# pingooio/pingoo

Measured on AMD Instinct MI355X. Metric: requests/sec matched (whole node), 1k-rule WAF, higher is better.
Workload: dtype u8

## Files before the change

include/pwaf.h:

```cpp
#ifndef PWAF_H
#define PWAF_H

#include <stddef.h>
#include <stdint.h>

#ifdef __cplusplus
extern "C" {
#endif

#define PWAF_ABI_VERSION 4u

#define PWAF_OK 0
#define PWAF_E_INVALID_ARG (-1)
#define PWAF_E_SYNTAX (-2)
#define PWAF_E_UNSUPPORTED (-3)
#define PWAF_E_LIST (-4)
#define PWAF_E_DEVICE (-5)
#define PWAF_E_BATCH (-6)
#define PWAF_E_NOMEM (-7)
#define PWAF_E_BUSY (-8)
#define PWAF_W_PARTIAL 1

#define PWAF_ACTION_ALLOW 0u
#define PWAF_ACTION_BLOCK 1u
// ... 417 lines not shown

typedef struct pwaf_kernel_time {
    char name[48];
    float ms;
    uint64_t alg_bytes;
} pwaf_kernel_time;
int pwaf_engine_set_profiling(pwaf_engine *, int on);
int pwaf_engine_kernel_times(pwaf_engine *, pwaf_kernel_time *out, int cap);

typedef struct pwaf_stats {
    uint32_t n_rules, n_atoms, n_scan_atoms, n_numeric_atoms;
    uint32_t n_dfa_groups, n_dfa_states_total, max_dfa_states, dfa_table_bytes_total;
    uint32_t n_ip_lists, ipset_trie_nodes, geo_trie_nodes, n_dnf_literals;
    uint32_t n_warnings, n_filtered_groups ,
        n_gated_groups ,
        n_confirm_literals ;
} pwaf_stats;
int pwaf_engine_stats(const pwaf_engine *, pwaf_stats *out);
int pwaf_engine_rule_errors(pwaf_engine *, uint64_t *counts, size_t n_rules);
int pwaf_engine_residual_mode(const pwaf_engine *);
const char *pwaf_engine_residual_fallback(const pwaf_engine *);
size_t pwaf_program_residual_source(const pwaf_program *, int kind, char *buf, size_t cap);
long pwaf_program_residual_compile(const pwaf_program *, const char *arch, char *err, size_t err_len);
int pwaf_program_confirm_field(const pwaf_program *, uint32_t group, const uint8_t *bytes, size_t len, uint32_t arena_offset,
                               uint16_t *atoms, size_t cap, size_t *n_atoms, int *flagged, int *walk);
int pwaf_program_confirm_shape(const pwaf_program *, uint32_t group, uint32_t out[8]);
size_t pwaf_program_flat_image(const pwaf_program *, uint32_t group, uint32_t tier, uint8_t *buf, size_t cap);
#define PWAF_LIST_SCAN_WORDS 16
int pwaf_program_list_scans(const pwaf_program *, uint32_t *out, size_t cap, size_t *n_descs);
int pwaf_program_verdict_shape(const pwaf_program *, uint32_t out[8]);
uint32_t pwaf_engine_compute_units(const pwaf_engine *);
int pwaf_engine_address_tables(const pwaf_engine *, uint32_t out[8]);
int pwaf_engine_coarse_tables(const pwaf_engine *, uint32_t out[16]);
#define PWAF_FILTER_SLAB_ROWS 128
int pwaf_engine_filter_flags(pwaf_engine *, uint32_t group, uint32_t info[8], uint64_t *rows, size_t cap_rows, uint32_t *per_slab, uint32_t *pair_base, size_t cap_slabs);
int pwaf_program_stats(const pwaf_program *, pwaf_stats *out);

size_t pwaf_derive_path(const uint8_t *uri_path, size_t len);
void pwaf_derive_user_agent(const uint8_t *hdr, size_t len, int present, size_t *out_start, size_t *out_len);
void pwaf_derive_host(const uint8_t *uri_host, size_t uri_host_len, int uri_host_present,
                      const uint8_t *host_hdr, size_t host_hdr_len, int host_hdr_present,
                      int *out_from_header, size_t *out_start, size_t *out_len);

const char *pwaf_last_error(void);
uint32_t pwaf_abi_version(void);

#ifdef __cplusplus
}
#endif
#endif
```

pingoo_amd/csrc/attr.hip:

```cpp
#include <hip/hip_runtime.h>

#include <algorithm>
#include <cstdlib>

#include "kernels.h"
#include "wave.h"

namespace pwaf {

static constexpr uint32_t DIR_ESCAPE = 0x80000000u;

__device__ __forceinline__ uint32_t ip_byte(const uint32_t w[4], uint32_t k) {
    uint32_t word = k < 4 ? w[0] : k < 8 ? w[1] : k < 12 ? w[2] : w[3];
    return (word >> ((k & 3) * 8)) & 0xFFu;
}

template <bool PACKED, bool COARSE>
__global__ __launch_bounds__(COARSE ? 1024 : 256, COARSE ? 8 : 1) void ipres_kernel(VerdictArgs a) {
    constexpr uint32_t U = 4;
    extern __shared__ uint4 ipres_lds[];
    const bool from_row = a.asn == nullptr;
#ifdef PWAF_PROFILING
    const bool dir = a.dir_chunks != nullptr && !((a.debug_skip >> 16) & 1u);
    const bool skip_v6 = (a.debug_skip >> 17) & 1u, skip_v4 = (a.debug_skip >> 16) & 1u;
#else
    const bool dir = a.dir_chunks != nullptr;
    constexpr bool skip_v6 = false, skip_v4 = false;
#endif
    const uint32_t T = gridDim.x * blockDim.x;
    uint32_t i0 = blockIdx.x * blockDim.x + threadIdx.x;
    uint4 raw[U];
    uint32_t v6b[U];
    auto load_inputs = [&](uint32_t base) {
#pragma unroll
        for (uint32_t u = 0; u < U; u++) {
            const uint32_t j = base + u * T < a.n ? base + u * T : base;
            raw[u] = *reinterpret_cast<const uint4 *>(a.ip + (size_t)j * 16);
            v6b[u] = a.ip_is_v6[j];
        }
    };
    bool loaded = false;
    if (COARSE) {
        load_inputs(i0 < a.n ? i0 : 0u);
        loaded = true;
        const uint4 *src = reinterpret_cast<const uint4 *>(a.dir_coarse);
        const uint32_t n16 = a.dir_coarse_bytes >> 4;
        for (uint32_t j = threadIdx.x; j < n16; j += 4u * blockDim.x) {
            uint4 w[4];
#pragma unroll
            for (uint32_t q = 0; q < 4; q++) w[q] = src[min(j + q * blockDim.x, n16 - 1u)];
#pragma unroll
            for (uint32_t q = 0; q < 4; q++)
                if (j + q * blockDim.x < n16) ipres_lds[j + q * blockDim.x] = w[q];
        }
        __syncthreads();
    }
    for (; i0 < a.n; i0 += T * U) {
        uint32_t idx[U], ipw[U][4], eg[U], ei[U], k[U];
        bool live[U], v6[U], geo_walk[U], chunked[U];
        if (!loaded) load_inputs(i0);
        loaded = false;
#pragma unroll
        for (uint32_t u = 0; u < U; u++) {
            idx[u] = i0 + u * T;
            live[u] = idx[u] < a.n;
        }
        uint32_t first[U], top16[U];
#pragma unroll
        for (uint32_t u = 0; u < U; u++) {
            ipw[u][0] = raw[u].x; ipw[u][1] = raw[u].y; ipw[u][2] = raw[u].z; ipw[u][3] = raw[u].w;
            v6[u] = v6b[u] != 0;
            geo_walk[u] = false;
            if (from_row && a.has_geo) {
                if (!v6[u]) {
                    const uint32_t b0 = ipw[u][0] & 0xFFu;
                    geo_walk[u] = !(b0 == 127u || (b0 & 0xF0u) == 0xE0u);
                } else {
                    const bool loopback = ipw[u][0] == 0 && ipw[u][1] == 0 && ipw[u][2] == 0 && ipw[u][3] == 0x01000000u;
                    geo_walk[u] = !(loopback || (ipw[u][0] & 0xFFu) == 0xFFu);
                }
            }
            top16[u] = (ip_byte(ipw[u], 0) << 8) | ip_byte(ipw[u], 1);
            eg[u] = ei[u] = TRIE_LEAF;
            chunked[u] = !v6[u] && dir;
            first[u] = 0;
            if (!chunked[u] && !(v6[u] ? skip_v6 : skip_v4)) {
                if (geo_walk[u]) eg[u] = (v6[u] ? a.geo_root6 : a.geo_root4)[top16[u]];
                if (a.n_ip_lists) ei[u] = (v6[u] ? a.ip_root6 : a.ip_root4)[top16[u]];
            }
        }
        uint32_t look[U];
#pragma unroll
        for (uint32_t u = 0; u < U; u++) {
            look[u] = chunked[u] ? 1u : 0u;
            if (COARSE && chunked[u]) {
                const uint32_t blk = ((top16[u] << 8) | ip_byte(ipw[u], 2)) >> a.dir_coarse_shift;
                look[u] = (reinterpret_cast<const uint32_t *>(ipres_lds)[blk >> 5] >> (blk & 31u)) & 1u;
            }
        }
#pragma unroll
        for (uint32_t u = 0; u < U; u++) {
            if (look[u] && a.dir_summary != nullptr) {
                const uint32_t blk = ((top16[u] << 8) | ip_byte(ipw[u], 2)) >> a.dir_sum_shift;
                look[u] = (a.dir_summary[blk >> 5] >> (blk & 31u)) & 1u;
            }
        }
        uint4 rec4[U];
#pragma unroll
        for (uint32_t u = 0; u < U; u++) {
            rec4[u] = make_uint4(0u, 0u, 0u, 0u);
            if (look[u]) rec4[u] = *reinterpret_cast<const uint4 *>(a.dir_chunks + (size_t)top16[u] * kDirChunkWords + 4u * (ip_byte(ipw[u], 2) >> 5));
        }
        uint32_t e24[U];
#pragma unroll
        for (uint32_t u = 0; u < U; u++) {
            e24[u] = a.dir_common;
            if (look[u]) {
                const uint32_t rank = (uint32_t)__builtin_popcount(rec4[u].x & (0xFFFFFFFFu >> (31u - (ip_byte(ipw[u], 2) & 31u))));
                e24[u] = rank == 0 ? rec4[u].y : rank == 1 ? rec4[u].z : a.dir_vals[rec4[u].w + rank - 2u];
            }
        }
#pragma unroll
        for (uint32_t u = 0; u < U; u++) {
            k[u] = 2;
            if (!v6[u] && dir) {
                k[u] = 3;
                if (e24[u] & DIR_ESCAPE) {
                    const uint2 esc = a.dir_esc[e24[u] & ~DIR_ESCAPE];
                    eg[u] = esc.x;
                    ei[u] = esc.y;
                } else {
                    eg[u] = TRIE_LEAF | (e24[u] & 0xFFFFu);
                    ei[u] = TRIE_LEAF | (e24[u] >> 16);
                }
            }
            if (!geo_walk[u]) eg[u] = TRIE_LEAF | a.geo_default;
            if (a.n_ip_lists == 0) ei[u] = TRIE_LEAF;
        }
        for (;;) {
            bool more = false;
#pragma unroll
            for (uint32_t u = 0; u < U; u++) more = more || !((eg[u] & ei[u]) & TRIE_LEAF);
            if (!more) break;
            uint32_t ng[U], ni[U];
#pragma unroll
            for (uint32_t u = 0; u < U; u++) {
                const uint32_t byte = ip_byte(ipw[u], k[u] < 16 ? k[u] : 15u);
                ng[u] = (eg[u] & TRIE_LEAF) ? eg[u] : a.geo_nodes[(size_t)eg[u] * 256 + byte];
                ni[u] = (ei[u] & TRIE_LEAF) ? ei[u] : a.ip_nodes[(size_t)ei[u] * 256 + byte];
            }
#pragma unroll
            for (uint32_t u = 0; u < U; u++) {
                if (!((eg[u] & ei[u]) & TRIE_LEAF)) k[u]++;
                eg[u] = ng[u];
                ei[u] = ni[u];
            }
        }
#pragma unroll
        for (uint32_t u = 0; u < U; u++) {
            if (!live[u]) continue;
            const uint32_t cls = eg[u] & ~TRIE_LEAF, set_id = ei[u] & ~TRIE_LEAF;
            if (PACKED) a.ipres[idx[u]] = cls | (set_id << 16);
            else reinterpret_cast<uint2 *>(a.ipres)[idx[u]] = make_uint2(cls, set_id);
        }
    }
}

__global__ __launch_bounds__(256) void georec_kernel(GeoRecArgs a) {
    constexpr uint32_t U = 4;
    const uint32_t T = gridDim.x * 256u;
    if (a.asn != nullptr) {
        for (uint32_t i = blockIdx.x * 256u + threadIdx.x; i < a.n; i += T) a.out[i] = make_uint2(a.asn[i], (uint32_t)a.country[i]);
        return;
    }
    const bool dir = a.chunks != nullptr;
    for (uint32_t i0 = blockIdx.x * 256u + threadIdx.x; i0 < a.n; i0 += T * U) {
        uint32_t idx[U], ipw[U][4], e[U], k[U], top16[U], v6b[U];
        bool live[U], chunked[U];
        uint4 raw[U];
#pragma unroll
        for (uint32_t u = 0; u < U; u++) {
            idx[u] = i0 + u * T;
            live[u] = idx[u] < a.n;
            const uint32_t j = live[u] ? idx[u] : i0;
            raw[u] = *reinterpret_cast<const uint4 *>(a.ip + (size_t)j * 16);
            v6b[u] = a.ip_is_v6[j];
        }
#pragma unroll
        for (uint32_t u = 0; u < U; u++) {
            ipw[u][0] = raw[u].x; ipw[u][1] = raw[u].y; ipw[u][2] = raw[u].z; ipw[u][3] = raw[u].w;
            const bool v6 = v6b[u] != 0;
            bool walk = a.has_geo != 0;
            if (!v6) {
                const uint32_t b0 = ipw[u][0] & 0xFFu;
                walk = walk && !(b0 == 127u || (b0 & 0xF0u) == 0xE0u);
            } else {
// ... 317 lines not shown
        c_slo = n_slo;
        c_shi = n_shi;
    }
}

__global__ __launch_bounds__(256) void dir24_kernel(VerdictArgs a, uint32_t *out, uint2 *esc, uint32_t *esc_count) {
    const uint32_t x = blockIdx.x * 256 + threadIdx.x;
    if (x >= (1u << 24)) return;
    uint32_t eg = a.geo_root4[x >> 8];
    if (!(eg & TRIE_LEAF)) eg = a.geo_nodes[(size_t)eg * 256 + (x & 0xFFu)];
    uint32_t ei = a.ip_root4[x >> 8];
    if (!(ei & TRIE_LEAF)) ei = a.ip_nodes[(size_t)ei * 256 + (x & 0xFFu)];
    const uint32_t vg = eg & ~TRIE_LEAF, vi = ei & ~TRIE_LEAF;
    if ((eg & ei & TRIE_LEAF) && vg < 65536u && vi < 32768u) {
        if (out) out[x] = vg | (vi << 16);
        return;
    }
    const uint32_t idx = atomicAdd(esc_count, 1u);
    if (esc) {
        esc[idx] = make_uint2(eg, ei);
        out[x] = DIR_ESCAPE | idx;
    }
}

int launch_dir24(const VerdictArgs &a, void *out, void *esc, void *esc_count, void *stream) {
    hipLaunchKernelGGL(dir24_kernel, dim3((1u << 24) / 256), dim3(256), 0, (hipStream_t)stream, a, (uint32_t *)out, (uint2 *)esc, (uint32_t *)esc_count);
    return (int)hipGetLastError();
}

#ifndef PWAF_IPRES_SHAPE
#define PWAF_IPRES_SHAPE 1
#endif
IpresShape ipres_shape() {
    static const IpresShape shapes[4] = {{256, 0, 8}, {1024, 64 * 1024, 2}, {512, 32 * 1024, 4}, {1024, 64 * 1024, 1}};
#ifdef PWAF_PROFILING
    static const uint32_t pick = getenv("PWAF_IPRES_SHAPE") ? (uint32_t)atoi(getenv("PWAF_IPRES_SHAPE")) & 3u : (uint32_t)PWAF_IPRES_SHAPE;
#else
    const uint32_t pick = PWAF_IPRES_SHAPE;
#endif
    return shapes[pick];
}

int launch_ipres(const VerdictArgs &a, void *stream) {
    if (a.n == 0) return 0;
#ifdef PWAF_PROFILING
    static const uint32_t forced = getenv("PWAF_IPRES_BLOCKS") ? (uint32_t)atoi(getenv("PWAF_IPRES_BLOCKS")) : 0u;
#else
    const uint32_t forced = 0;
#endif
    if (a.dir_coarse != nullptr) {
        const IpresShape sh = ipres_shape();
        if (a.dir_coarse_shift > 17u || a.dir_coarse_bytes != (1u << 21) >> a.dir_coarse_shift || a.dir_coarse_bytes > sh.coarse_bytes) return (int)hipErrorInvalidValue;
        const uint32_t blocks = std::min<uint32_t>((a.n + sh.threads - 1) / sh.threads, forced ? forced : sh.wg_per_cu * std::max(1u, a.attr_blocks));
        if (a.ipres_packed) hipLaunchKernelGGL((ipres_kernel<true, true>), dim3(blocks), dim3(sh.threads), a.dir_coarse_bytes, (hipStream_t)stream, a);
        else hipLaunchKernelGGL((ipres_kernel<false, true>), dim3(blocks), dim3(sh.threads), a.dir_coarse_bytes, (hipStream_t)stream, a);
        return (int)hipGetLastError();
    }
    const uint32_t blocks = std::min<uint32_t>((a.n + 255) / 256, forced ? forced : 8 * std::max(1u, a.attr_blocks));
    if (a.ipres_packed) hipLaunchKernelGGL((ipres_kernel<true, false>), dim3(blocks), dim3(256), 0, (hipStream_t)stream, a);
    else hipLaunchKernelGGL((ipres_kernel<false, false>), dim3(blocks), dim3(256), 0, (hipStream_t)stream, a);
    return (int)hipGetLastError();
}

int launch_georec(const GeoRecArgs &a, void *stream) {
    if (a.n == 0) return 0;
    const uint32_t blocks = std::min<uint32_t>((a.n + 255) / 256, 8 * std::max(1u, a.n_cus));
    hipLaunchKernelGGL(georec_kernel, dim3(blocks), dim3(256), 0, (hipStream_t)stream, a);
    return (int)hipGetLastError();
}

int launch_attr(const VerdictArgs &a, void *stream) {
    if (a.n == 0) return 0;
#ifdef PWAF_PROFILING
    static const uint32_t forced = getenv("PWAF_ATTR_BLOCKS") ? (uint32_t)atoi(getenv("PWAF_ATTR_BLOCKS")) : 0u;
#else
    const uint32_t forced = 0;
#endif
    const uint32_t blocks = std::min<uint32_t>((a.n_groups + 3) / 4, forced ? forced : 6 * std::max(1u, a.attr_blocks));
    const bool small = a.set_words <= 4 && a.cc_words <= 2 && a.iu_words[0] <= 1 && a.iu_words[1] <= 1 && a.acmp_words <= 1;
    if (a.ipres_packed && small) hipLaunchKernelGGL((attr_kernel<true, true>), dim3(blocks), dim3(256), 0, (hipStream_t)stream, a);
    else if (a.ipres_packed) hipLaunchKernelGGL((attr_kernel<true, false>), dim3(blocks), dim3(256), 0, (hipStream_t)stream, a);
    else if (small) hipLaunchKernelGGL((attr_kernel<false, true>), dim3(blocks), dim3(256), 0, (hipStream_t)stream, a);
    else hipLaunchKernelGGL((attr_kernel<false, false>), dim3(blocks), dim3(256), 0, (hipStream_t)stream, a);
    return (int)hipGetLastError();
}

}
```

pingoo_amd/csrc/engine.cpp:

```cpp
#include "dirtable.h"
#include "engine_impl.h"
#include "georec.h"

using namespace pwaf;

namespace {

Switches read_switches() {
    Switches s;
#ifdef PWAF_PROFILING
    const auto set = [](const char *name) { return getenv(name) != nullptr; };
    s.sync_each = set("PWAF_SYNC_EACH");
    if (set("PWAF_DEBUG_SKIP")) s.debug_skip = (uint32_t)strtoul(getenv("PWAF_DEBUG_SKIP"), nullptr, 0);
    s.attr_prio = set("PWAF_ATTR_PRIO");
    s.placement = set("PWAF_PLACEMENT") ? atoi(getenv("PWAF_PLACEMENT")) : set("PWAF_ATTR_INLINE") ? 1 : set("PWAF_ATTR_EARLY") ? 3 : 2;
    s.skip_attr = set("PWAF_SKIP_ATTR");
    s.skip_ipres = set("PWAF_SKIP_IPRES") || s.skip_attr;
    if (set("PWAF_LIST_SHAPE")) s.list_shape = (long)(uint32_t)atoi(getenv("PWAF_LIST_SHAPE"));
    if (set("PWAF_FILTER_DEBUG_SKIP")) s.filter_debug_skip = (uint32_t)atoi(getenv("PWAF_FILTER_DEBUG_SKIP"));
    s.attr_after_compact = set("PWAF_ATTR_AFTER_COMPACT");
    s.dump_counts = set("PWAF_DUMP_COUNTS");
    s.skip_identity = set("PWAF_SKIP_IDENTITY");
    s.side_priority_high = set("PWAF_SIDE_PRIORITY_HIGH");
    s.no_packed_staging = set("PWAF_NO_PACKED_STAGING");
// ... 374 lines not shown
int pwaf_engine_residual_mode(const pwaf_engine *e) {
    if (!e || e->prog.p->n_residual == 0) return 0;
    return e->residual_jit.function ? 2 : 1;
}
const char *pwaf_engine_residual_fallback(const pwaf_engine *e) { return e ? e->residual_note.c_str() : ""; }
int pwaf_engine_address_tables(const pwaf_engine *e, uint32_t out[8]) {
    if (!e || !out) return fail(PWAF_E_INVALID_ARG, "pwaf_engine_address_tables: NULL argument");
    const Program &P = *e->prog.p;
    VerdictArgs v{};
    set_trie_args(e, v);
    out[0] = e->dir_n_esc;
    out[1] = e->dir_chunks.p ? e->dir_n_vals : 0u;
    out[2] = e->dir_summary.p ? 1u : 0u;
    out[3] = e->dir_sum_shift;
    out[4] = e->dir_common;
    out[5] = v.ipres_packed;
    out[6] = e->n_classes;
    out[7] = P.set_words ? (uint32_t)(P.set_masks.size() / P.set_words) : 1u;
    return PWAF_OK;
}
int pwaf_engine_coarse_tables(const pwaf_engine *e, uint32_t out[16]) {
    if (!e || !out) return fail(PWAF_E_INVALID_ARG, "pwaf_engine_coarse_tables: NULL argument");
    const IpresShape sh = ipres_shape();
    for (int i = 0; i < 16; i++) out[i] = 0;
    out[0] = e->dir_coarse.p ? 1u : 0u;
    out[1] = e->dir_coarse_shift;
    out[2] = e->dir_coarse_bytes;
    out[3] = e->dir_coarse_set;
    out[4] = e->dir_summary_set;
    out[5] = e->dir_coarse.p ? sh.threads : 256u;
    out[6] = e->dir_coarse.p ? sh.wg_per_cu : 8u;
    return PWAF_OK;
}
int pwaf_engine_filter_flags(pwaf_engine *e, uint32_t group, uint32_t info[8], uint64_t *rows, size_t cap_rows, uint32_t *per_slab, uint32_t *pair_base, size_t cap_slabs) {
    if (!e || !info) return fail(PWAF_E_INVALID_ARG, "pwaf_engine_filter_flags: NULL argument");
    if (group >= e->groups.size() || !e->groups[group].filtered) return fail(PWAF_E_INVALID_ARG, "pwaf_engine_filter_flags: pass " + std::to_string(group) + " has no prefilter");
    HIP_TRY(hipSetDevice(e->device));
    Scratch *S = nullptr;
    for (auto &c : e->ctx) {
        std::lock_guard<std::mutex> lock(c->mu);
        if (!c->used || !(c->last_own || c->last == nullptr)) continue;
        if (S) return fail(PWAF_E_INVALID_ARG, "pwaf_engine_filter_flags: host batches and default-stream device batches were mixed on this engine: which came last is not recorded");
        S = c.get();
    }
    if (!S) return fail(PWAF_E_INVALID_ARG, "pwaf_engine_filter_flags: the engine has evaluated nothing");
    std::lock_guard<std::mutex> lock(S->mu);
    HIP_TRY(hipEventSynchronize(S->done));
    uint32_t fi = 0;
    for (uint32_t k = 0; k < group; k++) fi += e->groups[k].filtered ? 1u : 0u;
    for (int i = 0; i < 8; i++) info[i] = 0;
    info[2] = e->groups[group].filter.stride;
    info[3] = e->groups[group].confirm ? 1u : 0u;
    info[5] = PWAF_FILTER_SLAB_ROWS;
    static_assert(PWAF_FILTER_SLAB_ROWS == kStreamSlab / 1024, "one 64-bit word per KiB row of a slab");
    if (fi >= S->last_filter.size()) return PWAF_OK;
    const FilterArgs &f = S->last_filter[fi];
    const size_t slabs = (size_t)(((uint64_t)f.total + kStreamSlab - 1) / kStreamSlab) - f.slab0;
    info[0] = f.slab0;
    info[1] = (uint32_t)slabs;
    info[2] = f.stride;
    info[3] = f.pairs ? 1u : 0u;
    if ((rows && cap_rows < slabs * PWAF_FILTER_SLAB_ROWS) || ((per_slab || pair_base) && cap_slabs < slabs))
        return fail(PWAF_E_INVALID_ARG, "pwaf_engine_filter_flags: the pass streamed " + std::to_string(slabs) + " slabs, the arrays are shorter");
    if (f.pairs) HIP_TRY(hipMemcpy(&info[4], f.pair_count, 4, hipMemcpyDeviceToHost));
    if (!slabs) return PWAF_OK;
    if (rows) HIP_TRY(hipMemcpy(rows, f.chunk_bits, slabs * PWAF_FILTER_SLAB_ROWS * 8, hipMemcpyDeviceToHost));
// ... 108 lines not shown
```

pingoo_amd/csrc/engine_impl.h:

```cpp
#pragma once
#include <hip/hip_runtime_api.h>

#include <cstdio>
#include <algorithm>
#include <cstring>
#include <memory>
#include <mutex>
#include <string>
#include <vector>

#include "kernels.h"
#include "program_handle.h"
#include "scanplan.h"
#include "staging.h"
#include "tableplan.h"

#define HIP_TRY(expr)                                                                                              \
    do {                                                                                                           \
        hipError_t _e = (expr);                                                                                    \
        if (_e != hipSuccess) return pwaf::fail(PWAF_E_DEVICE, std::string(#expr) + ": " + hipGetErrorString(_e)); \
    } while (0)

#pragma GCC visibility push(hidden)
namespace pwaf {
// ... 160 lines not shown
            if (ev) (void)hipEventDestroy(ev);
        if (stream) (void)hipStreamDestroy(stream);
        if (side) (void)hipStreamDestroy(side);
        for (hipEvent_t ev : {ev_fork, ev_join, done})
            if (ev) (void)hipEventDestroy(ev);
    }
};
static constexpr size_t kContexts = 3;

struct pwaf_engine : pwaf::PlanShape, pwaf::PassShape {
    using DevBuf = pwaf::DevBuf;
    pwaf_program prog;
    int device = 0;
    std::vector<std::unique_ptr<Scratch>> ctx;
    size_t next_ctx = 0;
    std::vector<pwaf::DevGroup> groups;
    DevBuf num_atoms, bit_atoms , trig_off, trig_rules, always_rules, country_luts , rules, lits, set_masks;
    DevBuf lazy_atoms;
    DevBuf short_atoms;
    DevBuf class_rows, dir_esc, leaf_root, geo_leaf_root;
    DevBuf iu_vals[2], iu_masks[2];
    DevBuf ip_root4, ip_root6, ip_nodes, geo_root4, geo_root6, geo_nodes, geo_recs;
    std::mutex mu;
    std::mutex prof_mu;
    DevBuf residual_errors;
    std::string residual_note;
    pwaf::JitKernel residual_jit;
    DevBuf rules_unrouted;
    DevBuf residual_blob, geo_rec_root4, geo_rec_root6, geo_rec_nodes;
    DevBuf pass_base, colmask, dir24 , dir_chunks, dir_vals, dir_summary;
    uint32_t dir_sum_shift = 0, dir_common = 0;
    DevBuf dir_coarse;
    uint32_t dir_coarse_shift = 0, dir_coarse_bytes = 0, dir_coarse_set = 0, dir_summary_set = 0;
    uint32_t dir_n_esc = 0, dir_n_vals = 0;
    bool geo_answers = false;
    DevBuf georec_chunks, georec_vals, georec_summary;
    uint32_t georec_shift = 0, georec_common = 0, georec_n_esc = 0, georec_n_vals = 0;
    std::vector<double> mean_len;
    pwaf::ListPlan list_plan;
    DevBuf pass_table;
    uint32_t n_fields = PWAF_N_FIELDS;
    int profiling = 0;
    std::vector<hipEvent_t> ev;
    std::vector<pwaf_kernel_time> times;
    std::vector<std::pair<size_t, size_t>> time_ev;
    size_t n_timed = 0;
    uint32_t n_cus = 256;
};

namespace pwaf {


void set_trie_args(const pwaf_engine *e, VerdictArgs &v);
void set_georec_args(const pwaf_engine *e, GeoRecArgs &g);
int need_geo_answers(const pwaf_engine *e, const char *fn);
int need_routes(const pwaf_engine *e, const char *fn);

struct ReportOut {
    pwaf_rule_hit *hits = nullptr;
    uint32_t cap = 0;
    uint32_t *n_hits = nullptr;
    uint64_t *rule_hits = nullptr;
    uint32_t *route = nullptr;
    bool hit_any() const { return hits || n_hits || rule_hits; }
    bool any() const { return hit_any() || route; }
};
// ... 101 lines not shown
```

pingoo_amd/csrc/kernels.h:

```cpp
#pragma once
#include <cstdint>
#include <string>
#include <vector>

#include "program.h"
#include "scanplan.h"
#include "verdictplan.h"

namespace pwaf {

static constexpr int kMaxPasses = 250;
static constexpr int kVerdictPre = 12;
static constexpr uint32_t kDirChunkWords = 32;

static constexpr uint32_t REC_OVERFLOW = 0x80000000u;
struct PoolEntry {
    uint32_t atom;
    uint32_t next;
};

struct ScanArgs {
    const uint8_t *data;
    const uint32_t *off;
    uint32_t n;
// ... 269 lines not shown
    uint32_t iu_n[2], iu_words[2];
    const uint32_t *country_masks;
    uint32_t cc_words;
    const DevRule *rules;
    uint32_t n_rules;
    const uint32_t *lits;
    uint32_t n_lits, n_trig;
    const uint32_t *trig_off;
    const uint16_t *trig_rules;
    const uint32_t *always_rules;
    const uint32_t *ip_root4, *ip_root6, *ip_nodes;
    const uint32_t *set_masks;
    uint32_t set_words;
    uint32_t n_ip_lists;
    const uint32_t *geo_root4, *geo_root6, *geo_nodes;
    const uint32_t *dir24;
    const uint32_t *dir_chunks, *dir_vals;
    const uint32_t *dir_summary;
    uint32_t dir_sum_shift, dir_common;
    const uint32_t *dir_coarse;
    uint32_t dir_coarse_shift, dir_coarse_bytes;
    const uint2 *dir_esc;
    const uint32_t *class_rows;
    uint32_t class_words;
    uint32_t acmp_words;
    uint32_t geo_default;
    uint32_t *ipres;
    uint32_t ipres_packed;
    uint32_t has_geo;
    uint4 *gpairs;
    uint32_t *ghdr;
    uint32_t pair_stride;
    uint32_t attr_blocks;
    pwaf_verdict *out;
    unsigned long long *counts;
    uint32_t *match_idx;
    uint32_t *n_matches;
    pwaf_rule_hit *hits;
    uint32_t hits_cap;
    uint32_t *n_hits;
    unsigned long long *rule_hits;
    uint32_t *route;
    uint32_t route_base;
};

int launch_scan(const ScanArgs &a, void *stream);
struct GatedTable {
    const ListScanArgs *g;
    uint32_t count;
    uint32_t debug;
};
int launch_scan_gated(const ListScanArgs *host, uint32_t count, const ListScanArgs *dev, uint32_t *plan, const ListShape &shape, void *stream);
int launch_verdict(const VerdictArgs &a, void *stream);
int launch_ipres(const VerdictArgs &a, void *stream);
struct IpresShape {
    uint32_t threads, coarse_bytes, wg_per_cu;
};
IpresShape ipres_shape();
int launch_attr(const VerdictArgs &a, void *stream);
int launch_dir24(const VerdictArgs &a, void *out , void *esc, void *esc_count, void *stream);
struct GeoRecArgs {
    const uint8_t *ip, *ip_is_v6;
    const uint32_t *asn;
    const uint16_t *country;
    uint32_t n, has_geo;
    const uint32_t *root4, *root6, *nodes;
    const GeoRec *recs;
    const uint32_t *chunks, *vals, *summary;
    uint32_t sum_shift, common;
    uint32_t n_cus;
    uint2 *out;
};
int launch_georec(const GeoRecArgs &a, void *stream);
uint32_t scan_lds_bytes(uint32_t n_hot, uint32_t stride, uint32_t n_gate_atoms);

}
```

pingoo_amd/csrc/pipeline.cpp:

```cpp
#include <type_traits>

#include "engine_impl.h"
#include "georec.h"
#include "lscan_split.h"

using namespace pwaf;

namespace {

uint32_t slab_count(uint32_t total, uint32_t slab0) { return (uint32_t)(((uint64_t)total + kStreamSlab - 1) / kStreamSlab) - slab0; }
uint32_t slabs_of(const FilterArgs &f) { return slab_count(f.total, f.slab0); }
uint32_t pair_cap_of(uint32_t slabs, uint32_t n) { return (uint32_t)std::min<uint64_t>(0xFFFFFFF0u, (uint64_t)slabs * (kStreamSlab / 16) + n + 64); }

struct ArgSlotMark {
    Scratch &S;
    hipStream_t stream;
    int slot = -1;
    int record() {
        if (slot < 0) return PWAF_OK;
        const int k = slot;
        slot = -1;
        S.arg_pending[k] = true;
        HIP_TRY(hipEventRecord(S.arg_ev[k], stream));
        return PWAF_OK;
// ... 132 lines not shown
            const uint32_t spill_cols = entry_list ? P.n_cols : P.n_cols - std::min(vs.v_cap, P.n_cols);
            if (entry_list || spill_cols) {
                if ((rc = S.verdict_spill.reserve((size_t)verdict_blocks_sp(vs, e->n_cus) * vs.waves * spill_cols * 8))) return rc;
                v.spill = (unsigned long long *)S.verdict_spill.p;
            }
        }
        v.debug_skip = sw.debug_skip | (sw.attr_prio ? 0x80000000u : 0u);
        for (int f = 0; f < PWAF_N_FIELDS; f++) v.off[f] = db.field[f].offsets;
        v.ip = db.ip;
        v.ip_is_v6 = db.ip_is_v6;
        v.port = db.port;
        v.flags = db.flags;
        v.asn = db.asn;
        v.country = db.country;
        v.n_cols = P.n_cols;
        v.n_passes = n_passes;
        v.rec = (const uint32_t *)S.rec.p;
        v.passes = (const PassInfo *)e->pass_table.p;
        if (P.n_residual && e->residual_jit.function) {
            v.res_words = (P.n_residual + 31u) / 32u;
            v.res_base = P.residual_base;
            if ((rc = S.res_words.reserve((size_t)v.res_words * n * 4))) return rc;
            v.res_match = (const uint32_t *)S.res_words.p;
        }
        v.cand_bits = (const uint32_t *)S.cand_bits.p;
        v.visit_bits = (const uint32_t *)S.visit_bits.p;
        v.bit_words = bit_words;
        v.n_hlen = (uint32_t)e->hlen_fields.size();
        for (size_t k = 0; k < e->hlen_fields.size(); k++) v.hoff[k] = cols[e->hlen_fields[k]].offsets;
        v.gpairs = (uint4 *)S.attr.p;
        v.ghdr = (uint32_t *)((char *)S.attr.p + ((size_t)n_groups * pair_stride + 64) * 16);
        v.pair_stride = pair_stride;
        v.attr_blocks = e->n_cus;
        v.pool = (const PoolEntry *)S.pool.p;
        v.cmp = (const CmpAtomDev *)e->num_atoms.p;
        v.n_cmp = e->n_cmp_atoms;
        v.cmp_vars = e->cmp_vars;
        v.lazy = (const CmpAtomDev *)e->lazy_atoms.p;
        v.n_lazy = e->n_lazy;
        v.n_lazy_var = (uint32_t)e->lazy_vars.size();
        for (size_t k = 0; k < e->lazy_vars.size(); k++) v.lazy_var[k] = e->lazy_vars[k];
        v.n_short = e->n_short;
        v.short_atoms = (const ShortAtom *)e->short_atoms.p;
        if (e->n_short) {
            v.short_data = cols[(size_t)e->short_field].data;
            v.short_off = cols[(size_t)e->short_field].offsets;
        }
        v.n_trig = e->n_trig;
        v.n_lits = (uint32_t)P.lits.size();
        v.bit_col = (const uint32_t *)e->bit_atoms.p;
        v.trig_off = (const uint32_t *)e->trig_off.p;
        v.trig_rules = (const uint16_t *)e->trig_rules.p;
        v.always_rules = (const uint32_t *)e->always_rules.p;
        for (int var = 0; var < 2; var++) {
            v.iu_vals[var] = (const int64_t *)e->iu_vals[var].p;
            v.iu_masks[var] = (const uint32_t *)e->iu_masks[var].p;
            v.iu_n[var] = e->iu_n[var];
            v.iu_words[var] = e->iu_words[var];
        }
        v.country_masks = (const uint32_t *)e->country_luts.p;
        v.cc_words = e->cc_words;
        v.rules = (const DevRule *)e->rules.p;
        v.n_rules = (uint32_t)P.rules.size();
        v.lits = (const uint32_t *)e->lits.p;
        set_trie_args(e, v);
        if ((rc = S.ipres.reserve((size_t)n * (v.ipres_packed ? 4 : 8) + 64))) return rc;
// ... 629 lines not shown
```

pingoo_amd/engine.py:

```python
from __future__ import annotations

import ctypes as C
import enum
import ipaddress
import os
from dataclasses import dataclass, field
from typing import Dict, Iterable, List, Optional, Sequence, Tuple

import numpy as np

from . import _abi
from .batch import GEO_DTYPE, RESPONSE_DTYPE, RULE_HIT_DTYPE, VERDICT_DTYPE, Request, RequestBatch

_LIB = None
_LIB_PATH = os.path.join(os.path.dirname(os.path.abspath(__file__)), f"libpwaf_{os.environ['PWAF_LIB_VARIANT']}.so" if os.environ.get("PWAF_LIB_VARIANT") else "libpwaf.so")


class PwafError(RuntimeError):
    def __init__(self, code: int, message: str, rule_index: Optional[int] = None):
        super().__init__(f"[{code}] {message}")
        self.code = code
        self.message = message
        self.rule_index = rule_index

# ... 132 lines not shown
    L.pwaf_derive_scratch_bytes.restype = C.c_size_t
    L.pwaf_derive_batch.argtypes = [C.POINTER(_abi.Batch), C.POINTER(_abi.RawColumns), C.POINTER(_abi.DerivedCol), vp, vp, C.c_size_t, vp]
    L.pwaf_derive_scan_shape.argtypes = [C.POINTER(C.c_uint32)]
    L.pwaf_async_create.argtypes = [vp, C.c_uint32, C.c_uint32, C.c_uint32, C.POINTER(vp)]
    L.pwaf_async_submit.argtypes = [vp, C.POINTER(_abi.Request), C.c_uint64]
    L.pwaf_async_poll.argtypes = [vp, C.POINTER(_abi.Completion), C.c_size_t]
    L.pwaf_async_poll.restype = C.c_size_t
    L.pwaf_async_fd.argtypes = [vp]
    L.pwaf_async_flush.argtypes = [vp]
    L.pwaf_async_stats.argtypes = [vp, C.POINTER(C.c_uint64), C.POINTER(C.c_uint64), C.POINTER(C.c_uint64)]
    L.pwaf_async_destroy.argtypes = [vp]
    L.pwaf_async_destroy.restype = None
    L.pwaf_geoip_lookup.argtypes = [vp, vp, vp, C.c_uint32, C.c_uint32, vp, vp]
    L.pwaf_evaluate_batch_geo.argtypes = [vp, C.POINTER(_abi.Batch), vp, vp, vp]
    L.pwaf_evaluate_device_geo.argtypes = [vp, C.POINTER(_abi.Batch), vp, vp, vp, vp, vp, vp]
    L.pwaf_evaluate_batch_hits.argtypes = [vp, C.POINTER(_abi.Batch), vp, vp, vp, C.c_uint32, vp, vp]
    L.pwaf_evaluate_device_hits.argtypes = [vp, C.POINTER(_abi.Batch), vp, vp, vp, vp, vp, C.c_uint32, vp, vp, vp]
    routed_args = create_args[:2] + [C.POINTER(_abi.RouteDesc), C.c_size_t] + create_args[2:]
    L.pwaf_program_compile_routed.argtypes = routed_args + [C.POINTER(vp), C.POINTER(_abi.CompileError)]
    L.pwaf_engine_create_routed.argtypes = routed_args + [C.POINTER(vp), C.POINTER(_abi.CompileError)]
    for fn_name in ("pwaf_engine_route_count", "pwaf_program_route_count"):
        getattr(L, fn_name).argtypes = [vp]
        getattr(L, fn_name).restype = C.c_uint32
    L.pwaf_evaluate_batch_routes.argtypes = [vp, C.POINTER(_abi.Batch), vp, vp, vp]
    L.pwaf_evaluate_device_routes.argtypes = [vp, C.POINTER(_abi.Batch), vp, vp, vp, vp, vp, vp]
    L.pwaf_evaluate_one_route.argtypes = [vp, C.POINTER(_abi.Request), C.POINTER(_abi.Verdict), C.POINTER(C.c_uint32)]
    L.pwaf_evaluate_records_geo.argtypes = [vp, vp, C.c_size_t, vp, C.c_uint32, vp, vp, vp]
    L.pwaf_evaluate_one_geo.argtypes = [vp, C.POINTER(_abi.Request), C.POINTER(_abi.Verdict), C.POINTER(_abi.Geo)]
    L.pwaf_async_create_geo.argtypes = [vp, C.c_uint32, C.c_uint32, C.c_uint32, C.POINTER(vp)]
    L.pwaf_async_poll_geo.argtypes = [vp, C.POINTER(_abi.Completion), C.POINTER(_abi.Geo), C.c_size_t]
    L.pwaf_async_poll_geo.restype = C.c_size_t
    L.pwaf_engine_geo_answer_tables.argtypes = [vp, C.POINTER(C.c_uint32)]
    L.pwaf_engine_coarse_tables.argtypes = [vp, C.POINTER(C.c_uint32)]
    L.pwaf_engine_filter_flags.argtypes = [vp, C.c_uint32, C.POINTER(C.c_uint32), vp, C.c_size_t, vp, vp, C.c_size_t]
    L.pwaf_geoip_from_mmdb.argtypes = [C.c_char_p, C.c_size_t, C.POINTER(C.POINTER(_abi.GeoipEntry)), C.POINTER(C.c_size_t)]
    L.pwaf_geoip_from_file_image.argtypes = [C.c_char_p, C.c_char_p, C.c_size_t, C.POINTER(C.POINTER(_abi.GeoipEntry)), C.POINTER(C.c_size_t)]
    L.pwaf_zstd_decompress.argtypes = [C.c_char_p, C.c_size_t, C.POINTER(C.c_void_p), C.POINTER(C.c_size_t)]
    L.pwaf_buffer_free.argtypes = [C.c_void_p]
    L.pwaf_buffer_free.restype = None
    L.pwaf_geoip_free.argtypes = [C.POINTER(_abi.GeoipEntry)]
    L.pwaf_geoip_free.restype = None
    L.pwaf_list_parse_csv.argtypes = [C.c_char_p, C.c_size_t, C.POINTER(C.POINTER(C.c_char_p)), C.POINTER(C.c_size_t)]
    L.pwaf_list_free.argtypes = [C.POINTER(C.c_char_p), C.c_size_t]
    L.pwaf_list_free.restype = None
    L.pwaf_engine_kernel_times.argtypes = [vp, C.POINTER(_abi.KernelTime), C.c_int]
    L.pwaf_derive_path.argtypes = [C.c_char_p, C.c_size_t]
    L.pwaf_derive_path.restype = C.c_size_t
    L.pwaf_derive_user_agent.argtypes = [C.c_char_p, C.c_size_t, C.c_int, C.POINTER(C.c_size_t), C.POINTER(C.c_size_t)]
    L.pwaf_derive_user_agent.restype = None
    L.pwaf_derive_host.argtypes = [C.c_char_p, C.c_size_t, C.c_int, C.c_char_p, C.c_size_t, C.c_int, C.POINTER(C.c_int), C.POINTER(C.c_size_t), C.POINTER(C.c_size_t)]
    L.pwaf_derive_host.restype = None
    if L.pwaf_abi_version() != _abi.ABI_VERSION:
        raise ImportError("libpwaf.so ABI version mismatch: rebuild with `python -m pingoo_amd.build --force`")
    _LIB = L
    return L


def _raise(code: int, message: str, rule_index: Optional[int] = None):
    cls = {_abi.E_SYNTAX: ExpressionIsNotValid, _abi.E_UNSUPPORTED: UnsupportedExpression, _abi.E_DEVICE: DeviceError}.get(code, PwafError)
    raise cls(code, message, rule_index)


def _check(rc: int, message: str = "", rule_index: Optional[int] = None) -> None:
    if rc != 0:
        _raise(rc, message or lib().pwaf_last_error().decode(errors="replace"), rule_index)

# ... 237 lines not shown

    def close(self):
        if getattr(self, "_h", None):
            lib().pwaf_engine_destroy(self._h)
            self._h = None

    def __del__(self):
        self.close()

    @property
    def program(self) -> CompiledProgram:
        return CompiledProgram._borrow(lib().pwaf_engine_program(self._h))

    @property
    def residual_mode(self) -> int:
        return int(lib().pwaf_engine_residual_mode(self._h))

    @property
    def residual_fallback(self) -> str:
        return (lib().pwaf_engine_residual_fallback(self._h) or b"").decode(errors="replace")

    def compute_units(self) -> int:
        return int(lib().pwaf_engine_compute_units(self._h))

    def address_tables(self) -> dict:
        out = (C.c_uint32 * len(_abi.ADDRESS_TABLE_FIELDS))()
        _check(lib().pwaf_engine_address_tables(self._h, out))
        return dict(zip(_abi.ADDRESS_TABLE_FIELDS, (int(x) for x in out)))

    def coarse_tables(self) -> dict:
        out = (C.c_uint32 * len(_abi.COARSE_TABLE_FIELDS))()
        _check(lib().pwaf_engine_coarse_tables(self._h, out))
        return dict(zip(_abi.COARSE_TABLE_FIELDS, (int(x) for x in out)))

    def filter_flags(self, group: int) -> dict:
        L = lib()
        info = (C.c_uint32 * len(_abi.FILTER_FLAGS_FIELDS))()
        _check(L.pwaf_engine_filter_flags(self._h, group, info, None, 0, None, None, 0))
        d = dict(zip(_abi.FILTER_FLAGS_FIELDS, (int(x) for x in info)))
        assert d["slab_rows"] == _abi.FILTER_SLAB_ROWS
        slabs = d["slabs"]
        rows = np.zeros(slabs * _abi.FILTER_SLAB_ROWS, dtype="<u8")
        per_slab, pair_base = np.zeros(slabs, dtype=np.uint32), np.zeros(slabs, dtype=np.uint32)
        if slabs:
            _check(L.pwaf_engine_filter_flags(self._h, group, info, rows.ctypes.data, len(rows), per_slab.ctypes.data, pair_base.ctypes.data, slabs))
        has_pairs = bool(d["has_pairs"])
        return dict(slab0=d["slab0"], slabs=slabs, stride=d["stride"], chunks=np.unpackbits(rows.view(np.uint8), bitorder="little").astype(bool), per_slab=per_slab,
                    pair_base=pair_base if has_pairs else None, pair_count=d["pair_count"] if has_pairs else None)

    def geo_answer_tables(self) -> dict:
        out = (C.c_uint32 * len(_abi.GEO_ANSWER_TABLE_FIELDS))()
        _check(lib().pwaf_engine_geo_answer_tables(self._h, out))
        return dict(zip(_abi.GEO_ANSWER_TABLE_FIELDS, (int(x) for x in out)))

    def lookup_geoip(self, ip16, v6) -> np.ndarray:
        ip16 = np.ascontiguousarray(ip16, dtype=np.uint8).reshape(-1, 16)
        v6 = np.ascontiguousarray(v6, dtype=np.uint8).reshape(-1)
        assert len(ip16) == len(v6)
        out = np.zeros(len(v6), dtype=GEO_DTYPE)
        _check(lib().pwaf_geoip_lookup(self._h, ip16.ctypes.data, v6.ctypes.data, len(v6), _abi.MEM_HOST, out.ctypes.data, None))
        return out

    def rule_errors(self, n_rules: int) -> List[int]:
        arr = (C.c_uint64 * n_rules)()
        _check(lib().pwaf_engine_rule_errors(self._h, arr, n_rules))
        return list(arr)
# ... 1100 lines not shown
```

Baseline: 7.911 billion.

## Batch IP-resolution table loads and add optional next-tile input prefetch variant

Restructures the IP resolution kernel so each table lookup stage issues all U gathers before consuming them, using compiler barriers and a byte-swapped 24-bit prefix for simpler address math. Adds an AHEAD template variant (768-thread shape) that prefetches the next iteration's inputs during the summary lookup. Also adds an API to override the lookup workgroup count. The prefetch variant is only selected by a non-default shape, and holding extra in-flight registers may reduce occupancy.

```diff
diff --git a/include/pwaf.h b/include/pwaf.h
--- a/include/pwaf.h
+++ b/include/pwaf.h
@@ -473,6 +473,7 @@
 uint32_t pwaf_engine_compute_units(const pwaf_engine *);
 int pwaf_engine_address_tables(const pwaf_engine *, uint32_t out[8]);
 int pwaf_engine_coarse_tables(const pwaf_engine *, uint32_t out[16]);
+int pwaf_engine_set_lookup_workgroups(pwaf_engine *, uint32_t workgroups);
 #define PWAF_FILTER_SLAB_ROWS 128
 int pwaf_engine_filter_flags(pwaf_engine *, uint32_t group, uint32_t info[8], uint64_t *rows, size_t cap_rows, uint32_t *per_slab, uint32_t *pair_base, size_t cap_slabs);
 int pwaf_program_stats(const pwaf_program *, pwaf_stats *out);
diff --git a/pingoo_amd/csrc/attr.hip b/pingoo_amd/csrc/attr.hip
--- a/pingoo_amd/csrc/attr.hip
+++ b/pingoo_amd/csrc/attr.hip
@@ -15,8 +15,13 @@
     return (word >> ((k & 3) * 8)) & 0xFFu;
 }
 
-template <bool PACKED, bool COARSE>
-__global__ __launch_bounds__(COARSE ? 1024 : 256, COARSE ? 8 : 1) void ipres_kernel(VerdictArgs a) {
+template <class T>
+__device__ __forceinline__ T gather32(const void *base, uint32_t byte_off) {
+    return *reinterpret_cast<const T *>(static_cast<const char *>(base) + byte_off);
+}
+
+template <bool PACKED, bool COARSE, bool AHEAD>
+__global__ __launch_bounds__(COARSE ? (AHEAD ? 768 : 1024) : 256, COARSE ? (AHEAD ? 6 : 8) : 1) void ipres_kernel(VerdictArgs a) {
     constexpr uint32_t U = 4;
     extern __shared__ uint4 ipres_lds[];
     const bool from_row = a.asn == nullptr;
@@ -31,18 +36,17 @@
     uint32_t i0 = blockIdx.x * blockDim.x + threadIdx.x;
     uint4 raw[U];
     uint32_t v6b[U];
-    auto load_inputs = [&](uint32_t base) {
+    auto load_inputs = [&](uint32_t base, uint4 (&r)[U], uint32_t (&f)[U]) {
 #pragma unroll
         for (uint32_t u = 0; u < U; u++) {
             const uint32_t j = base + u * T < a.n ? base + u * T : base;
-            raw[u] = *reinterpret_cast<const uint4 *>(a.ip + (size_t)j * 16);
-            v6b[u] = a.ip_is_v6[j];
+            r[u] = *reinterpret_cast<const uint4 *>(a.ip + (size_t)j * 16);
+            f[u] = a.ip_is_v6[j];
         }
     };
-    bool loaded = false;
+    const bool have_sum = dir && a.dir_summary != nullptr;
+    load_inputs(i0 < a.n ? i0 : 0u, raw, v6b);
     if (COARSE) {
-        load_inputs(i0 < a.n ? i0 : 0u);
-        loaded = true;
         const uint4 *src = reinterpret_cast<const uint4 *>(a.dir_coarse);
         const uint32_t n16 = a.dir_coarse_bytes >> 4;
         for (uint32_t j = threadIdx.x; j < n16; j += 4u * blockDim.x) {
@@ -55,17 +59,15 @@
         }
         __syncthreads();
     }
+    bool loaded = true;
     for (; i0 < a.n; i0 += T * U) {
-        uint32_t idx[U], ipw[U][4], eg[U], ei[U], k[U];
-        bool live[U], v6[U], geo_walk[U], chunked[U];
-        if (!loaded) load_inputs(i0);
+        uint32_t ipw[U][4], eg[U], ei[U], k[U];
+        if (!AHEAD && !loaded) load_inputs(i0, raw, v6b);
         loaded = false;
 #pragma unroll
-        for (uint32_t u = 0; u < U; u++) {
-            idx[u] = i0 + u * T;
-            live[u] = idx[u] < a.n;
-        }
-        uint32_t first[U], top16[U];
+        for (uint32_t u = 0; u < U; u++) asm volatile("" : "+v"(raw[u].x), "+v"(raw[u].y), "+v"(raw[u].z), "+v"(raw[u].w), "+v"(v6b[u]));
+        bool v6[U], geo_walk[U], chunked[U];
+        uint32_t h24[U];
 #pragma unroll
         for (uint32_t u = 0; u < U; u++) {
             ipw[u][0] = raw[u].x; ipw[u][1] = raw[u].y; ipw[u][2] = raw[u].z; ipw[u][3] = raw[u].w;
@@ -80,55 +82,73 @@
                     geo_walk[u] = !(loopback || (ipw[u][0] & 0xFFu) == 0xFFu);
                 }
             }
-            top16[u] = (ip_byte(ipw[u], 0) << 8) | ip_byte(ipw[u], 1);
+            h24[u] = __builtin_bswap32(ipw[u][0]) >> 8;
             eg[u] = ei[u] = TRIE_LEAF;
             chunked[u] = !v6[u] && dir;
-            first[u] = 0;
             if (!chunked[u] && !(v6[u] ? skip_v6 : skip_v4)) {
-                if (geo_walk[u]) eg[u] = (v6[u] ? a.geo_root6 : a.geo_root4)[top16[u]];
-                if (a.n_ip_lists) ei[u] = (v6[u] ? a.ip_root6 : a.ip_root4)[top16[u]];
+                const uint32_t root_off = (h24[u] >> 6) & ~3u;
+                if (geo_walk[u]) eg[u] = gather32<uint32_t>(v6[u] ? a.geo_root6 : a.geo_root4, root_off);
+                if (a.n_ip_lists) ei[u] = gather32<uint32_t>(v6[u] ? a.ip_root6 : a.ip_root4, root_off);
             }
         }
         uint32_t look[U];
-#pragma unroll
-        for (uint32_t u = 0; u < U; u++) {
-            look[u] = chunked[u] ? 1u : 0u;
-            if (COARSE && chunked[u]) {
-                const uint32_t blk = ((top16[u] << 8) | ip_byte(ipw[u], 2)) >> a.dir_coarse_shift;
-                look[u] = (reinterpret_cast<const uint32_t *>(ipres_lds)[blk >> 5] >> (blk & 31u)) & 1u;
-            }
-        }
-#pragma unroll
-        for (uint32_t u = 0; u < U; u++) {
-            if (look[u] && a.dir_summary != nullptr) {
-                const uint32_t blk = ((top16[u] << 8) | ip_byte(ipw[u], 2)) >> a.dir_sum_shift;
-                look[u] = (a.dir_summary[blk >> 5] >> (blk & 31u)) & 1u;
-            }
-        }
+        if (COARSE) {
+            uint32_t cw[U];
+#pragma unroll
+            for (uint32_t u = 0; u < U; u++) cw[u] = reinterpret_cast<const uint32_t *>(ipres_lds)[chunked[u] ? h24[u] >> (a.dir_coarse_shift + 5u) : 0u];
+            asm volatile("" : "+v"(cw[0]), "+v"(cw[1]), "+v"(cw[2]), "+v"(cw[3]));
+#pragma unroll
+            for (uint32_t u = 0; u < U; u++) look[u] = chunked[u] ? (cw[u] >> ((h24[u] >> a.dir_coarse_shift) & 31u)) & 1u : 0u;
+        } else {
+#pragma unroll
+            for (uint32_t u = 0; u < U; u++) look[u] = chunked[u] ? 1u : 0u;
+        }
+        uint32_t sw[U];
+#pragma unroll
+        for (uint32_t u = 0; u < U; u++) {
+            sw[u] = ~0u;
+            if (look[u] && have_sum) sw[u] = gather32<uint32_t>(a.dir_summary, (h24[u] >> (a.dir_sum_shift + 5u)) << 2);
+        }
+        uint4 nraw[U];
+        uint32_t nv6[U];
+        if (AHEAD) {
+            const uint32_t nx = i0 + T * U;
+            load_inputs(nx < a.n && nx > i0 ? nx : i0, nraw, nv6);
+        }
+        asm volatile("" : "+v"(sw[0]), "+v"(sw[1]), "+v"(sw[2]), "+v"(sw[3]));
+#pragma unroll
+        for (uint32_t u = 0; u < U; u++) look[u] &= sw[u] >> ((h24[u] >> a.dir_sum_shift) & 31u);
         uint4 rec4[U];
 #pragma unroll
         for (uint32_t u = 0; u < U; u++) {
             rec4[u] = make_uint4(0u, 0u, 0u, 0u);
-            if (look[u]) rec4[u] = *reinterpret_cast<const uint4 *>(a.dir_chunks + (size_t)top16[u] * kDirChunkWords + 4u * (ip_byte(ipw[u], 2) >> 5));
-        }
-        uint32_t e24[U];
-#pragma unroll
-        for (uint32_t u = 0; u < U; u++) {
-            e24[u] = a.dir_common;
-            if (look[u]) {
-                const uint32_t rank = (uint32_t)__builtin_popcount(rec4[u].x & (0xFFFFFFFFu >> (31u - (ip_byte(ipw[u], 2) & 31u))));
-                e24[u] = rank == 0 ? rec4[u].y : rank == 1 ? rec4[u].z : a.dir_vals[rec4[u].w + rank - 2u];
-            }
-        }
+            if (look[u]) rec4[u] = gather32<uint4>(a.dir_chunks, (h24[u] >> 1) & ~15u);
+        }
+        uint32_t rank[U], val[U], e24[U];
+#pragma unroll
+        for (uint32_t u = 0; u < U; u++) {
+            rank[u] = (uint32_t)__builtin_popcount(rec4[u].x & (0xFFFFFFFFu >> (31u - (h24[u] & 31u))));
+            val[u] = 0;
+            if (rank[u] >= 2u) val[u] = gather32<uint32_t>(a.dir_vals, (rec4[u].w + rank[u] - 2u) << 2);
+        }
+        asm volatile("" : "+v"(val[0]), "+v"(val[1]), "+v"(val[2]), "+v"(val[3]));
+#pragma unroll
+        for (uint32_t u = 0; u < U; u++) e24[u] = !look[u] ? a.dir_common : rank[u] == 0 ? rec4[u].y : rank[u] == 1 ? rec4[u].z : val[u];
+        uint2 esc[U];
+#pragma unroll
+        for (uint32_t u = 0; u < U; u++) {
+            esc[u] = make_uint2(0u, 0u);
+            if (chunked[u] && (e24[u] & DIR_ESCAPE)) esc[u] = gather32<uint2>(a.dir_esc, (e24[u] & ~DIR_ESCAPE) << 3);
+        }
+        asm volatile("" : "+v"(esc[0].x), "+v"(esc[0].y), "+v"(esc[1].x), "+v"(esc[1].y), "+v"(esc[2].x), "+v"(esc[2].y), "+v"(esc[3].x), "+v"(esc[3].y));
 #pragma unroll
         for (uint32_t u = 0; u < U; u++) {
             k[u] = 2;
-            if (!v6[u] && dir) {
+            if (chunked[u]) {
                 k[u] = 3;
                 if (e24[u] & DIR_ESCAPE) {
-                    const uint2 esc = a.dir_esc[e24[u] & ~DIR_ESCAPE];
-                    eg[u] = esc.x;
-                    ei[u] = esc.y;
+                    eg[u] = esc[u].x;
+                    ei[u] = esc[u].y;
                 } else {
                     eg[u] = TRIE_LEAF | (e24[u] & 0xFFFFu);
                     ei[u] = TRIE_LEAF | (e24[u] >> 16);
@@ -158,10 +178,18 @@
         }
 #pragma unroll
         for (uint32_t u = 0; u < U; u++) {
-            if (!live[u]) continue;
+            const uint32_t idx = i0 + u * T;
+            if (idx >= a.n) continue;
             const uint32_t cls = eg[u] & ~TRIE_LEAF, set_id = ei[u] & ~TRIE_LEAF;
-            if (PACKED) a.ipres[idx[u]] = cls | (set_id << 16);
-            else reinterpret_cast<uint2 *>(a.ipres)[idx[u]] = make_uint2(cls, set_id);
+            if (PACKED) a.ipres[idx] = cls | (set_id << 16);
+            else reinterpret_cast<uint2 *>(a.ipres)[idx] = make_uint2(cls, set_id);
+        }
+        if (AHEAD) {
+#pragma unroll
+            for (uint32_t u = 0; u < U; u++) {
+                raw[u] = nraw[u];
+                v6b[u] = nv6[u];
+            }
         }
     }
 }
@@ -545,9 +573,9 @@
 #define PWAF_IPRES_SHAPE 1
 #endif
 IpresShape ipres_shape() {
-    static const IpresShape shapes[4] = {{256, 0, 8}, {1024, 64 * 1024, 2}, {512, 32 * 1024, 4}, {1024, 64 * 1024, 1}};
+    static const IpresShape shapes[5] = {{256, 0, 8, 0}, {1024, 64 * 1024, 2, 0}, {512, 32 * 1024, 4, 0}, {1024, 64 * 1024, 1, 0}, {768, 64 * 1024, 2, 1}};
 #ifdef PWAF_PROFILING
-    static const uint32_t pick = getenv("PWAF_IPRES_SHAPE") ? (uint32_t)atoi(getenv("PWAF_IPRES_SHAPE")) & 3u : (uint32_t)PWAF_IPRES_SHAPE;
+    static const uint32_t pick = getenv("PWAF_IPRES_SHAPE") ? std::min(4u, (uint32_t)atoi(getenv("PWAF_IPRES_SHAPE"))) : (uint32_t)PWAF_IPRES_SHAPE;
 #else
     const uint32_t pick = PWAF_IPRES_SHAPE;
 #endif
@@ -556,22 +584,27 @@
 
 int launch_ipres(const VerdictArgs &a, void *stream) {
     if (a.n == 0) return 0;
+    uint32_t forced = a.ipres_blocks;
 #ifdef PWAF_PROFILING
-    static const uint32_t forced = getenv("PWAF_IPRES_BLOCKS") ? (uint32_t)atoi(getenv("PWAF_IPRES_BLOCKS")) : 0u;
-#else
-    const uint32_t forced = 0;
+    static const uint32_t env_forced = getenv("PWAF_IPRES_BLOCKS") ? (uint32_t)atoi(getenv("PWAF_IPRES_BLOCKS")) : 0u;
+    if (!forced) forced = env_forced;
 #endif
     if (a.dir_coarse != nullptr) {
         const IpresShape sh = ipres_shape();
         if (a.dir_coarse_shift > 17u || a.dir_coarse_bytes != (1u << 21) >> a.dir_coarse_shift || a.dir_coarse_bytes > sh.coarse_bytes) return (int)hipErrorInvalidValue;
         const uint32_t blocks = std::min<uint32_t>((a.n + sh.threads - 1) / sh.threads, forced ? forced : sh.wg_per_cu * std::max(1u, a.attr_blocks));
-        if (a.ipres_packed) hipLaunchKernelGGL((ipres_kernel<true, true>), dim3(blocks), dim3(sh.threads), a.dir_coarse_bytes, (hipStream_t)stream, a);
-        else hipLaunchKernelGGL((ipres_kernel<false, true>), dim3(blocks), dim3(sh.threads), a.dir_coarse_bytes, (hipStream_t)stream, a);
+        if (sh.ahead) {
+            if (a.ipres_packed) hipLaunchKernelGGL((ipres_kernel<true, true, true>), dim3(blocks), dim3(sh.threads), a.dir_coarse_bytes, (hipStream_t)stream, a);
+            else hipLaunchKernelGGL((ipres_kernel<false, true, true>), dim3(blocks), dim3(sh.threads), a.dir_coarse_bytes, (hipStream_t)stream, a);
+        } else {
+            if (a.ipres_packed) hipLaunchKernelGGL((ipres_kernel<true, true, false>), dim3(blocks), dim3(sh.threads), a.dir_coarse_bytes, (hipStream_t)stream, a);
+            else hipLaunchKernelGGL((ipres_kernel<false, true, false>), dim3(blocks), dim3(sh.threads), a.dir_coarse_bytes, (hipStream_t)stream, a);
+        }
         return (int)hipGetLastError();
     }
     const uint32_t blocks = std::min<uint32_t>((a.n + 255) / 256, forced ? forced : 8 * std::max(1u, a.attr_blocks));
-    if (a.ipres_packed) hipLaunchKernelGGL((ipres_kernel<true, false>), dim3(blocks), dim3(256), 0, (hipStream_t)stream, a);
-    else hipLaunchKernelGGL((ipres_kernel<false, false>), dim3(blocks), dim3(256), 0, (hipStream_t)stream, a);
+    if (a.ipres_packed) hipLaunchKernelGGL((ipres_kernel<true, false, false>), dim3(blocks), dim3(256), 0, (hipStream_t)stream, a);
+    else hipLaunchKernelGGL((ipres_kernel<false, false, false>), dim3(blocks), dim3(256), 0, (hipStream_t)stream, a);
     return (int)hipGetLastError();
 }
 
diff --git a/pingoo_amd/csrc/engine.cpp b/pingoo_amd/csrc/engine.cpp
--- a/pingoo_amd/csrc/engine.cpp
+++ b/pingoo_amd/csrc/engine.cpp
@@ -430,6 +430,12 @@
     out[6] = e->dir_coarse.p ? sh.wg_per_cu : 8u;
     return PWAF_OK;
 }
+int pwaf_engine_set_lookup_workgroups(pwaf_engine *e, uint32_t workgroups) {
+    if (!e) return fail(PWAF_E_INVALID_ARG, "pwaf_engine_set_lookup_workgroups: NULL argument");
+    std::lock_guard<std::mutex> lock(e->mu);
+    e->ipres_blocks = workgroups;
+    return PWAF_OK;
+}
 int pwaf_engine_filter_flags(pwaf_engine *e, uint32_t group, uint32_t info[8], uint64_t *rows, size_t cap_rows, uint32_t *per_slab, uint32_t *pair_base, size_t cap_slabs) {
     if (!e || !info) return fail(PWAF_E_INVALID_ARG, "pwaf_engine_filter_flags: NULL argument");
     if (group >= e->groups.size() || !e->groups[group].filtered) return fail(PWAF_E_INVALID_ARG, "pwaf_engine_filter_flags: pass " + std::to_string(group) + " has no prefilter");
diff --git a/pingoo_amd/csrc/engine_impl.h b/pingoo_amd/csrc/engine_impl.h
--- a/pingoo_amd/csrc/engine_impl.h
+++ b/pingoo_amd/csrc/engine_impl.h
@@ -216,6 +216,7 @@
     uint32_t dir_sum_shift = 0, dir_common = 0;
     DevBuf dir_coarse;
     uint32_t dir_coarse_shift = 0, dir_coarse_bytes = 0, dir_coarse_set = 0, dir_summary_set = 0;
+    uint32_t ipres_blocks = 0;
     uint32_t dir_n_esc = 0, dir_n_vals = 0;
     bool geo_answers = false;
     DevBuf georec_chunks, georec_vals, georec_summary;
diff --git a/pingoo_amd/csrc/kernels.h b/pingoo_amd/csrc/kernels.h
--- a/pingoo_amd/csrc/kernels.h
+++ b/pingoo_amd/csrc/kernels.h
@@ -325,6 +325,7 @@
     uint32_t *ghdr;
     uint32_t pair_stride;
     uint32_t attr_blocks;
+    uint32_t ipres_blocks;
     pwaf_verdict *out;
     unsigned long long *counts;
     uint32_t *match_idx;
@@ -347,7 +348,7 @@
 int launch_verdict(const VerdictArgs &a, void *stream);
 int launch_ipres(const VerdictArgs &a, void *stream);
 struct IpresShape {
-    uint32_t threads, coarse_bytes, wg_per_cu;
+    uint32_t threads, coarse_bytes, wg_per_cu, ahead;
 };
 IpresShape ipres_shape();
 int launch_attr(const VerdictArgs &a, void *stream);
diff --git a/pingoo_amd/csrc/pipeline.cpp b/pingoo_amd/csrc/pipeline.cpp
--- a/pingoo_amd/csrc/pipeline.cpp
+++ b/pingoo_amd/csrc/pipeline.cpp
@@ -188,6 +188,7 @@
         v.ghdr = (uint32_t *)((char *)S.attr.p + ((size_t)n_groups * pair_stride + 64) * 16);
         v.pair_stride = pair_stride;
         v.attr_blocks = e->n_cus;
+        v.ipres_blocks = e->ipres_blocks;
         v.pool = (const PoolEntry *)S.pool.p;
         v.cmp = (const CmpAtomDev *)e->num_atoms.p;
         v.n_cmp = e->n_cmp_atoms;
diff --git a/pingoo_amd/engine.py b/pingoo_amd/engine.py
--- a/pingoo_amd/engine.py
+++ b/pingoo_amd/engine.py
@@ -188,6 +188,7 @@
     L.pwaf_async_poll_geo.restype = C.c_size_t
     L.pwaf_engine_geo_answer_tables.argtypes = [vp, C.POINTER(C.c_uint32)]
     L.pwaf_engine_coarse_tables.argtypes = [vp, C.POINTER(C.c_uint32)]
+    L.pwaf_engine_set_lookup_workgroups.argtypes = [vp, C.c_uint32]
     L.pwaf_engine_filter_flags.argtypes = [vp, C.c_uint32, C.POINTER(C.c_uint32), vp, C.c_size_t, vp, vp, C.c_size_t]
     L.pwaf_geoip_from_mmdb.argtypes = [C.c_char_p, C.c_size_t, C.POINTER(C.POINTER(_abi.GeoipEntry)), C.POINTER(C.c_size_t)]
     L.pwaf_geoip_from_file_image.argtypes = [C.c_char_p, C.c_char_p, C.c_size_t, C.POINTER(C.POINTER(_abi.GeoipEntry)), C.POINTER(C.c_size_t)]
@@ -491,6 +492,9 @@
         out = (C.c_uint32 * len(_abi.COARSE_TABLE_FIELDS))()
         _check(lib().pwaf_engine_coarse_tables(self._h, out))
         return dict(zip(_abi.COARSE_TABLE_FIELDS, (int(x) for x in out)))
+
+    def set_lookup_workgroups(self, workgroups: int) -> None:
+        _check(lib().pwaf_engine_set_lookup_workgroups(self._h, workgroups))
 
     def filter_flags(self, group: int) -> dict:
         L = lib()
```

Result: no change. 7.925 billion (median of 2 runs) (+0.2%).
